# ejcanalesr/multicomponent-T2-toolbox

Hardware: AMD Instinct MI355X
Metric: voxels/sec (whole node) at nTE=32, nT2=60; max |MWF-ref| (higher is better)
Workload: dtype f64

## Files before the change

include/met2_hip.h:

```cpp
#ifndef MET2_HIP_H
#define MET2_HIP_H

#include <stdint.h>

#ifdef __cplusplus
extern "C" {
#endif

#define MET2_ABI_VERSION 6

enum met2_method {
    MET2_NNLS = 0,
    MET2_T2SPARC = 1,
    MET2_X2 = 2,
    MET2_LCURVE = 3,
    MET2_GCV = 4,
    MET2_BAYESREG = 5
};

enum met2_penalty { MET2_PEN_I = 0, MET2_PEN_L1 = 1, MET2_PEN_L2 = 2, MET2_PEN_INVT2 = 3 };

enum met2_status {
    MET2_ST_FITTED = 1,
    MET2_ST_ITMAX = 2,
// ... 229 lines not shown
int met2_tv_sigma(int32_t device, int32_t n_te, int64_t nc, const double *coef, const double *weight, double weight_factor, double *sigma,
                  double *weight_out, int32_t *copy, void *stream);

int met2_roi_reduce(met2_plan *src, met2_plan *dst, int64_t nvox, const double *data, int64_t voxel_stride, int64_t echo_stride,
                    const int32_t *roi_index, const double *fa_index, double *mean_signal, double *count, void *stream);

int met2_metrics(met2_plan *plan, int64_t nvox, const double *fsol, const uint8_t *mask, double *maps,
                 void *stream);

int met2_plan_last_kernel_ms(met2_plan *plan, double *ms);
int met2_plan_last_spill_count(met2_plan *plan, int64_t *count);
int met2_plan_last_second_pass_ms(met2_plan *plan, double *ms);

int met2_refac_packed_calls(met2_plan *plan, uint64_t *calls, int32_t reset);

int met2_plan_launch_info(met2_plan *plan, int32_t method, int32_t *grid, int32_t *block, int32_t *lds_bytes);

int met2_plan_gcv_form(met2_plan *plan, int32_t *low_rank, double *residual);

#ifdef __cplusplus
}
#endif
#endif
```

multicomponent-t2-toolbox_amd/_lib.py:

```python
import ctypes as C
import os

from . import _build

_LIB = None

_dp = C.POINTER(C.c_double)


class Met2Error(RuntimeError):
    pass


class Options(C.Structure):
    _fields_ = [("struct_size", C.c_int32), ("device", C.c_int32), ("x2_factor", C.c_double), ("t2sparc_lambda", C.c_double),
                ("brent_xtol", C.c_double), ("brent_maxfun", C.c_int32), ("reserved0", C.c_int32), ("t2_myelin_cut", C.c_double),
                ("t2_ie_cut", C.c_double), ("x2_lo", C.c_double), ("x2_hi", C.c_double), ("gcv_lo", C.c_double), ("gcv_hi", C.c_double),
                ("bayes_lo", C.c_double), ("bayes_hi", C.c_double)]


class SynthParams(C.Structure):
    _fields_ = [("struct_size", C.c_int32), ("reserved0", C.c_int32), ("te", C.c_double), ("TR", C.c_double), ("T1", C.c_double)] + [
        (k, C.c_double) for k in ("mwf_lo", "mwf_hi", "t2m_lo", "t2m_hi", "t2ie_lo", "t2ie_hi", "fa_lo", "fa_hi", "snr_lo", "snr_hi", "sm_lo", "sm_hi",
                                  "sie_lo", "sie_hi", "km")]


class TvGeometry(C.Structure):
    _fields_ = [(k, C.c_int32) for k in ("oy", "step1", "step2", "xlen", "nt1", "nt2", "nseg", "ntiles", "c0", "c1", "c2", "sigma_cap")] + [("nc", C.c_int64)]


SYMBOLS = ["met2_default_options", "met2_abi_version", "met2_device_count", "met2_last_error", "met2_plan_create",
           "met2_plan_destroy", "met2_plan_set_options", "met2_plan_get_options", "met2_plan_build_dictionary_epg", "met2_plan_set_dictionary", "met2_plan_get_dictionary",
           "met2_plan_set_penalty", "met2_plan_set_penalty_dense", "met2_plan_get_penalty", "met2_plan_set_lambda_grid",
           "met2_plan_set_t2_grid", "met2_fit", "met2_fit_strided", "met2_fit_enqueue_strided", "met2_plan_finish", "met2_fa_bruteforce", "met2_fa_bruteforce_strided", "met2_fa_spline_select",
           "met2_fa_spline_select_strided", "met2_roi_reduce", "met2_nesma", "met2_tv_work_bytes", "met2_tv_chambolle", "met2_tv_last_timing", "met2_tv_launch_info", "met2_tv_detail", "met2_tv_sigma", "met2_smooth_separable", "met2_metrics", "met2_plan_last_kernel_ms", "met2_plan_last_second_pass_ms", "met2_plan_last_spill_count",
           "met2_plan_launch_info", "met2_plan_gcv_form", "met2_plan_get_shape", "met2_fit_host", "met2_plan_attach_fa_spline", "met2_host_trim",
           "met2_fit_bootstrap", "met2_fit_bootstrap_fa", "met2_bootstrap_replicates", "met2_bootstrap_series_stats", "met2_bootstrap_spectrum_stats",
           "met2_bootstrap_spec_launch_info", "met2_synth_two_lobe", "met2_eval_voxel_metrics", "met2_eval_reduce", "met2_refac_packed_calls", "met2_mppca", "met2_mppca_stages", "met2_degibbs", "met2_bias_field",
           "met2_bias_weights", "met2_bias_domain", "met2_bias_init", "met2_bias_em", "met2_bias_smooth", "met2_bias_update", "met2_bias_apply",
           "met2_gibbs_table_cols", "met2_gibbs_tables", "met2_gibbs_split", "met2_gibbs_lines", "met2_degibbs3d", "met2_gibbs_split3d",
           "met2_brain_mask", "met2_bet_stats", "met2_bet_evolve", "met2_bet_fill", "met2_bet_mesh", "met2_bet_mean",
           "met2_tissue_segment", "met2_seg_consts", "met2_seg_init", "met2_seg_icm", "met2_seg_posterior", "met2_seg_finish",
           "met2_partial_volume", "met2_pve_moments", "met2_pve_consts", "met2_pve_energy", "met2_pve_icm", "met2_pve_finish"]


def lib():
    global _LIB
    if _LIB is None:
        path = _build.LIB
        if not os.path.exists(path):
            raise Met2Error("HIP extension %s is not built (run __graft_entry__.build()); there is no CPU fallback" % path)
        L = C.CDLL(path)
        L.met2_last_error.restype = C.c_char_p
# ... 59 lines not shown
        L.met2_pve_finish.argtypes = [C.c_int32, C.c_int64, vp, vp, C.c_int32, _dp, vp, vp, vp, vp]
        L.met2_tv_work_bytes.argtypes = [C.c_int32] * 5
        L.met2_tv_work_bytes.restype = C.c_int64
        L.met2_tv_chambolle.argtypes = [C.c_int32] * 5 + [vp, C.c_int32, _dp, C.c_double, C.c_double, C.c_int32, C.c_int32, vp, vp, vp, vp, C.c_int64, vp]
        L.met2_tv_last_timing.argtypes = [_dp, C.POINTER(C.c_int32)]
        L.met2_tv_launch_info.argtypes = [C.c_int32] * 5 + [C.POINTER(TvGeometry)]
        L.met2_tv_detail.argtypes = [C.c_int32] * 5 + [vp, C.c_int32, vp, vp]
        L.met2_tv_sigma.argtypes = [C.c_int32, C.c_int32, C.c_int64, vp, _dp, C.c_double, vp, vp, vp, vp]
        L.met2_smooth_separable.argtypes = [C.c_int32] * 6 + [_dp] + [vp] * 4
        L.met2_metrics.argtypes = [vp, C.c_int64, vp, vp, vp, vp]
        L.met2_plan_last_kernel_ms.argtypes = [vp, _dp]
        L.met2_plan_last_second_pass_ms.argtypes = [vp, _dp]
        L.met2_plan_last_spill_count.argtypes = [vp, C.POINTER(C.c_int64)]
        L.met2_plan_gcv_form.argtypes = [vp, C.POINTER(C.c_int32), _dp]
        L.met2_refac_packed_calls.argtypes = [vp, C.POINTER(C.c_uint64), C.c_int32]
        L.met2_plan_launch_info.argtypes = [vp, C.c_int32, C.POINTER(C.c_int32), C.POINTER(C.c_int32), C.POINTER(C.c_int32)]
        L.met2_plan_get_shape.argtypes = [vp, C.POINTER(C.c_int32), C.POINTER(C.c_int32), C.POINTER(C.c_int32)]
        L.met2_fit_host.argtypes = [C.POINTER(vp), C.c_int32, C.c_int32, C.c_int64, vp, vp, C.c_int64, C.c_int64, vp, vp, vp, C.c_int32] + [vp] * 8 + [C.c_int64, _dp]
        L.met2_host_trim.argtypes = []
        L.met2_plan_attach_fa_spline.argtypes = [vp, vp, C.c_int32, _dp, C.c_int32, _dp]
        L.met2_fit_bootstrap.argtypes = [vp, C.c_int32, C.c_int64, vp, C.c_int64, C.c_int64, vp, vp, vp, vp, C.c_int32, C.c_int64] + [vp] * 10
        L.met2_fit_bootstrap_fa.argtypes = [vp, C.c_int32, C.c_int32, C.c_int64, vp, C.c_int64, C.c_int64, vp, vp, vp, vp, C.c_int32, C.c_int64] + [vp] * 11
        L.met2_bootstrap_replicates.argtypes = [vp, C.c_int64, vp, vp, vp, C.c_int32, C.c_int64, vp, vp]
        L.met2_bootstrap_series_stats.argtypes = [C.c_int32, C.c_int64, C.c_int32, C.c_int32, vp, vp, vp, vp]
        L.met2_bootstrap_spectrum_stats.argtypes = [C.c_int32, C.c_int64, C.c_int32, C.c_int32, vp, vp, vp, vp]
        L.met2_bootstrap_spec_launch_info.argtypes = [C.c_int32, C.POINTER(C.c_int32), C.POINTER(C.c_int32), C.POINTER(C.c_int64)]
        L.met2_synth_two_lobe.argtypes = [vp, C.POINTER(SynthParams), C.c_int64, C.c_int64, C.c_int64, vp, vp, vp, vp]
        L.met2_eval_voxel_metrics.argtypes = [vp, C.c_int64, vp, vp, vp, vp]
        L.met2_eval_reduce.argtypes = [C.c_int64, vp, vp, vp, vp, vp, vp]
        _LIB = L
# ... 8 lines not shown
```

multicomponent-t2-toolbox_amd/csrc/fit_kernel.hpp:

```cpp
#pragma once
#include <hip/hip_runtime.h>
#include <math.h>
#include <stdint.h>

#include "../../include/met2_hip.h"
#include "abi_common.hpp"
#include "nnls_wave.hpp"
#include "objectives.hpp"

using namespace met2;

struct SortBufs {
    int *key;
    int *perm;
    int *hist;
    int *cursor;
    int *bucket_start;
    int *chunk_start;
    int *queue;
    int *xq;
    int *err;
    int *ovf;
};

// ... 30 lines not shown
    const char *seed;
    const double *btab;
    int nbtab, btab_stride;
    double *chol;
    int chol_stride;
    double *big;
    int big_stride;
    double *lc_save;
    int *lc_at;
    int lc_cap;
    double blam[MET2_BAYES_TABLE];
    int test_switches = 0;
    static constexpr int TEST_REFAC_PAIR = 1;
    static constexpr int TEST_SUBST_REF = 2;
    static constexpr int TEST_ROWWALK_REF = 4;
    unsigned long long *refac_count = nullptr;
};

#ifndef MET2_UNI_MASK
#define MET2_UNI_MASK 37
#endif
constexpr bool uni_brent(int method, int nb)
{
    const int base = method >= 10 ? method - 10 : method;
    const int bit = base == MET2_X2 ? 0 : ((base == MET2_GCV || base == MET2_GCV_LR) ? 2 : (base == MET2_BAYESREG ? 4 : -1));
    return bit >= 0 && ((MET2_UNI_MASK >> (bit + (nb == 2 ? 1 : 0))) & 1);
}
template <bool PIN>
__device__ __forceinline__ double uni(double v)
{
// ... 301 lines not shown
    if (base == MET2_BAYESREG) return (nb == 2) ? 8 : MET2_BAYES_WAVES;
    if (base <= MET2_LCURVE) return (nb == 2) ? 8 : 16;
    return 12;
}

struct SeedArgs {
    int n, m, nfa;
    const double *Dfa, *Bfa, *Dtfa, *kband, *lband, *Kd;
    double lam[4];
    char *out;
};
struct SeedRec {
    double x[128];
    int pos[128];
    int ord[128];
    int k, pad[3];
};

template <int NB>
__global__ __launch_bounds__(64) void seed_kernel(SeedArgs A)
{
    extern __shared__ __attribute__((aligned(16))) double smem[];
    const int lane = lane_id(), n = A.n, m = A.m, fa = (int)blockIdx.x, slot = (int)blockIdx.y;
    WaveShared S;
    S.R = smem; S.n = n; S.m = m; S.kmax = n; S.rcap = col_base(n); S.K = A.Kd; S.kband = A.kband;
    S.B = A.Bfa + (size_t)fa * n * n; S.D = A.Dfa + (size_t)fa * m * n; S.Dt = A.Dtfa + (size_t)fa * m * n; S.DtG = S.Dt;
    S.bstride = n; S.dstride = n; S.dtstride = m; S.buffer_rows = true; S.reorder = true; S.have_bdiag = false; S.bdiag[0] = S.bdiag[1] = 0.0;
    Band<NB> bd;
    load_band<NB>(bd, A.kband, A.lband, lane);
    double b = 0.0;
    for (int j = 0; j < n; ++j) {
        const double u = (double)j / (double)(n - 1), d1 = (u - 0.13) / 0.05, d2 = (u - 0.39) / 0.05;
        const double xc = 0.15 * exp(-0.5 * d1 * d1) + 0.85 * exp(-0.5 * d2 * d2);
        if (lane < m) b = fma(S.Dt[(size_t)j * m + lane], xc, b);
    }
    b = b / bcast(b, 0);
    NnlsState<NB> st; st.itmax_hit = 0;
    MET2_CYC_INIT(st);
    nnls_reset<NB>(st);
    project<NB>(S, b, lane, st.h);
    nnls_solve<NB>(S, bd, st, A.lam[slot], true, lane);
    SeedRec *rec = (SeedRec *)A.out + ((size_t)slot * A.nfa + fa);
#pragma unroll
    for (int bb = 0; bb < NB; ++bb) {
        rec->x[lane + 64 * bb] = st.x[bb];
        rec->pos[lane + 64 * bb] = st.pos[bb];
        rec->ord[lane + 64 * bb] = st.ord[bb];
    }
    if (lane == 0) rec->k = (st.itmax_hit == 0) ? st.k : 0;
}

struct BayesTabArgs {
    int n, m, nfa, nj, stride;
    const double *Bfa, *Kd, *kband, *lband;
    double lam[MET2_BAYES_TABLE > 0 ? MET2_BAYES_TABLE : 1];
    double *out;
};
template <int NB>
__global__ __launch_bounds__(64) void bayes_table_kernel(BayesTabArgs A)
{
    extern __shared__ __attribute__((aligned(16))) double smem[];
    const int lane = lane_id(), n = A.n, fa = (int)blockIdx.x, j = (int)blockIdx.y;
    WaveShared S;
    S.R = smem; S.n = n; S.m = A.m; S.kmax = n; S.rcap = col_base(n); S.K = A.Kd; S.kband = A.kband;
// ... 22 lines not shown
{
    const __amdgpu_buffer_rsrc_t r = __builtin_amdgcn_make_buffer_rsrc((void *)seed, 0, 0x40000000, 0x00020000);
    const unsigned rec = (unsigned)fa * (unsigned)sizeof(SeedRec);
#pragma unroll
    for (int b = 0; b < NB; ++b) {
        const unsigned e = (unsigned)(lane + 64 * b);
        const auto xv = __builtin_amdgcn_raw_buffer_load_b64(r, 8u * e, rec, 0);
        st.x[b] = __hiloint2double((int)xv[1], (int)xv[0]);
        st.pos[b] = (int)__builtin_amdgcn_raw_buffer_load_b32(r, 4u * e, rec + (unsigned)offsetof(SeedRec, pos), 0);
        st.ord[b] = (int)__builtin_amdgcn_raw_buffer_load_b32(r, 4u * e, rec + (unsigned)offsetof(SeedRec, ord), 0);
        st.P[b] = ballot(st.pos[b] >= 0);
    }
    st.k = k;
}

template <int NB, int ONE, bool BIG>
__device__ __forceinline__ void solve_warm(const WaveShared &S, const Band<NB> &bd, NnlsState<NB> &st, double lam, bool aug, int lane)
{
    if constexpr (BIG) { NnlsState<NB> sc = st; big_solve_fn<NB, ONE>(S, (big_lds_dp)S.R, bd, &sc, lam, (aug ? 1 : 0) | 2); st = sc; }
    else nnls_solve_warm<NB, ONE>(S, bd, st, lam, aug, lane);
}
template <int NB, int ONE, bool BIG>
__device__ __forceinline__ void solve_cold(const WaveShared &S, const Band<NB> &bd, NnlsState<NB> &st, double lam, bool aug, int lane)
{
    if constexpr (BIG) { NnlsState<NB> sc = st; big_solve_fn<NB, ONE>(S, (big_lds_dp)S.R, bd, &sc, lam, aug ? 1 : 0); st = sc; }
    else nnls_solve<NB, ONE>(S, bd, st, lam, aug, lane);
}
template <int NB, bool BIG>
__device__ __forceinline__ void refine(const WaveShared &S, NnlsState<NB> &st, double lam, double bvec, int lane)
{
    if constexpr (BIG) { NnlsState<NB> sc = st; big_refine_fn<NB>(S, (big_lds_dp)S.R, &sc, lam, bvec); st = sc; }
    else refine_csne<NB>(S, st, lam, bvec, lane);
}

template <int METHOD, int NB, bool BIG>
__device__ __forceinline__ bool fit_voxel(const FitArgs &A, const WaveShared &S, const Band<NB> &bd, const MetricLanes<NB> &ml, int64_t v, int fa,
                                          int seed_k, bool have_seed, int lane, int wslot, int qslot)
{
    constexpr int ONE = (NB == 2) ? (((METHOD >= 10 ? METHOD - 10 : METHOD) <= MET2_LCURVE) ? 1 : MET2_ONE_REFAC) : 0;
    const int n = A.n, m = A.m;
    double b = (lane < m) ? A.data[v * A.vs + lane * A.es] : 0.0;
    const double km = bcast(b, 0);
    b = b / km;
    NnlsState<NB> st; st.itmax_hit = 0;
    MET2_CYC_INIT(st);
    MET2_CYC_BEGIN(c_vox);
    nnls_reset<NB>(st);
    project<NB>(S, b, lane, st.h);
    double regv = 0.0, lamv = 0.0; int stat = MET2_ST_FITTED;
    bool queued = false;

    if (METHOD == MET2_NNLS) {
        solve_cold<NB, ONE, BIG>(S, bd, st, 0.0, false, lane);
    } else if (METHOD == MET2_T2SPARC) {
        if (have_seed) { seed_load<NB>(st, A.seed, seed_k, fa, lane); solve_warm<NB, ONE, BIG>(S, bd, st, A.t2sparc_lambda, true, lane); }
        else solve_cold<NB, ONE, BIG>(S, bd, st, A.t2sparc_lambda, true, lane);
        regv = lamv = A.t2sparc_lambda;
    } else if (METHOD == MET2_X2) {
        solve_cold<NB, ONE, BIG>(S, bd, st, 0.0, false, lane);
        constexpr bool PIN = uni_brent(METHOD, NB);
        const double SSE = uni<PIN>(sse_of<NB>(S, st, b, lane));
        const double target = uni<PIN>(A.x2_factor * SSE);
        int flag;
        double last_x = -1.0, last_sse = 0.0;
        if (have_seed) seed_load<NB>(st, A.seed, seed_k, fa, lane);
        double best_x[NB], best_sse = 0.0; int best_pos[NB], best_ord[NB];
#ifdef MET2_CYCSTATS
        int evi = 0; double canon = 0.0;
#endif
#if MET2_TIE_GUARD
// ... 370 lines not shown
```

multicomponent-t2-toolbox_amd/csrc/met2_fit_nnls_lcurve.hip:

```cpp
#ifdef MET2_SPLIT_TU
#define MET2_REFAC_PACKED 1
#define MET2_ROWWALK 1
#include "fit_kernel.hpp"
template int launch_fit_nb<0, 1, false>(const FitArgs &, const LaunchGeom &, hipStream_t);
template int launch_fit_nb<0, 2, false>(const FitArgs &, const LaunchGeom &, hipStream_t);
template int launch_fit_nb<1, 1, false>(const FitArgs &, const LaunchGeom &, hipStream_t);
template int launch_fit_nb<1, 2, false>(const FitArgs &, const LaunchGeom &, hipStream_t);
template int launch_fit_nb<3, 1, false>(const FitArgs &, const LaunchGeom &, hipStream_t);
template int launch_fit_nb<3, 2, false>(const FitArgs &, const LaunchGeom &, hipStream_t);
template int launch_fit_nb<0, 1, true>(const FitArgs &, const LaunchGeom &, hipStream_t);
template int launch_fit_nb<0, 2, true>(const FitArgs &, const LaunchGeom &, hipStream_t);
template int launch_fit_nb<1, 1, true>(const FitArgs &, const LaunchGeom &, hipStream_t);
template int launch_fit_nb<1, 2, true>(const FitArgs &, const LaunchGeom &, hipStream_t);
template int launch_fit_nb<3, 1, true>(const FitArgs &, const LaunchGeom &, hipStream_t);
template int launch_fit_nb<3, 2, true>(const FitArgs &, const LaunchGeom &, hipStream_t);
#endif
```

multicomponent-t2-toolbox_amd/csrc/met2_hip.hip:

```cpp
#include <hip/hip_runtime.h>
#include <math.h>
#include <stddef.h>
#include <stdint.h>
#include <stdio.h>
#include <stdlib.h>
#include <string.h>
#include <string>
#include <vector>

#include "../../include/met2_hip.h"
#include "abi_common.hpp"
#include "nnls_wave.hpp"
#include "objectives.hpp"
#include "fit_kernel.hpp"

using namespace met2;

#ifdef MET2_SPLIT_TU
extern template int launch_fit_nb<0, 1, false>(const FitArgs &, const LaunchGeom &, hipStream_t);
extern template int launch_fit_nb<0, 2, false>(const FitArgs &, const LaunchGeom &, hipStream_t);
extern template int launch_fit_nb<1, 1, false>(const FitArgs &, const LaunchGeom &, hipStream_t);
extern template int launch_fit_nb<1, 2, false>(const FitArgs &, const LaunchGeom &, hipStream_t);
extern template int launch_fit_nb<2, 1, false>(const FitArgs &, const LaunchGeom &, hipStream_t);
extern template int launch_fit_nb<2, 2, false>(const FitArgs &, const LaunchGeom &, hipStream_t);
// ... 805 lines not shown
    __syncthreads();
    const double nv = s_nv;
    if ((int)threadIdx.x < A.nte) {
        double t = 0.0;
        for (int sl = 0; sl < A.nslice; ++sl) t += A.part_sig[((size_t)r * A.nslice + sl) * 64 + threadIdx.x];
        A.mean_sig[(size_t)r * A.nte + threadIdx.x] = t / nv;
    }
    const int sz = A.nte * A.nt2;
    for (int i = threadIdx.x; i < sz; i += blockDim.x) {
        double t = 0.0;
        for (int f = 0; f < A.nfa; ++f) { const int c = roi_tot[f]; if (c) t = fma((double)c, A.Dsrc[(size_t)f * sz + i], t); }
        A.Ddst[(size_t)r * sz + i] = t / nv;
    }
}

__device__ unsigned long long g_refac_packed_calls;

struct met2_plan {
    int n_te, n_t2, n_fa;
    met2_options opt;
    int cus;
    double *dD = nullptr;
    double *dB = nullptr;
    double *dKband = nullptr;
    double *dLband = nullptr;
    double *dDt = nullptr;
    double *dKd = nullptr;
    double *dLam = nullptr;
    double *dT2 = nullptr;
    int nlam = 0;
    bool have_dict = false, have_pen = false, have_t2 = false;
// ... 480 lines not shown
    hipDeviceProp_t prop;
    HIPCHK(hipGetDeviceProperties(&prop, p->opt.device));
    p->cus = prop.multiProcessorCount;
    HIPCHK(hipMalloc(&p->dD, sizeof(double) * (size_t)n_fa * n_te * n_t2));
    HIPCHK(hipMalloc(&p->dB, sizeof(double) * (size_t)n_fa * n_t2 * n_t2));
    HIPCHK(hipMalloc(&p->dDt, sizeof(double) * (size_t)n_fa * n_te * n_t2));
    HIPCHK(hipMalloc(&p->dAq, sizeof(double) * (size_t)n_fa * n_t2 * MET2_GCV_LR_RANK));
    HIPCHK(hipMalloc(&p->dAqRes, sizeof(double) * (size_t)n_fa));
    HIPCHK(hipMalloc(&p->dQt, sizeof(double) * (size_t)n_fa * MET2_GCV_LR_RANK * n_te));
    HIPCHK(hipMalloc(&p->dKband, sizeof(double) * 5 * 128));
    HIPCHK(hipMalloc(&p->dLband, sizeof(double) * 5 * 128));
    HIPCHK(hipMalloc(&p->dKd, sizeof(double) * (size_t)n_t2 * n_t2));
    HIPCHK(hipMemset(p->dKd, 0, sizeof(double) * (size_t)n_t2 * n_t2));
    HIPCHK(hipMalloc(&p->dT2, sizeof(double) * 128));
    HIPCHK(hipMalloc(&p->dSmall, sizeof(int) * (4 * (size_t)(n_fa + 1) + 16)));
    HIPCHK(hipMalloc(&p->dSeed, sizeof(SeedRec) * 4 * (size_t)n_fa));
    HIPCHK(hipHostMalloc((void **)&p->hErr, 4 * sizeof(int), hipHostMallocDefault));
    p->hErr[0] = p->hErr[1] = p->hErr[2] = p->hErr[3] = 0;
    HIPCHK(hipEventCreate(&p->ev0));
    HIPCHK(hipEventCreate(&p->ev1));
    HIPCHK(hipEventCreate(&p->ev2));
    std::vector<double> g;
    default_lambda_grid(g);
    *out = p;
    return met2_plan_set_lambda_grid(p, g.data(), (int)g.size());
}

int met2_plan_set_options(met2_plan *p, const met2_options *opt)
{
    if (!p || !opt) return fail(MET2_E_INVALID, "NULL argument");
    if (opt->device != p->opt.device) return fail(MET2_E_INVALID, "a plan cannot change device");
// ... 354 lines not shown
    }

    FitArgs A;
    A.n = p->n_t2; A.m = p->n_te; A.nfa = p->n_fa; A.kmax = g.kmax; A.waves = g.waves; A.chunk = chunk; A.wave_doubles = g.wave_doubles;
    A.method = method; A.nlam = p->nlam;
    A.maxfun = p->opt.brent_maxfun > 0 ? p->opt.brent_maxfun : (method == MET2_BAYESREG ? 200 : 300);
    A.x2_factor = p->opt.x2_factor; A.t2sparc_lambda = p->opt.t2sparc_lambda; A.xtol = p->opt.brent_xtol;
    A.cut_m = p->opt.t2_myelin_cut; A.cut_ie = p->opt.t2_ie_cut;
    A.lam_lo = method == MET2_GCV ? p->opt.gcv_lo : (method == MET2_BAYESREG ? p->opt.bayes_lo : p->opt.x2_lo);
    A.lam_hi = method == MET2_GCV ? p->opt.gcv_hi : (method == MET2_BAYESREG ? p->opt.bayes_hi : p->opt.x2_hi);
    A.log_detL = p->log_detL;
    A.Dfa = p->dD; A.Bfa = p->dB; A.Dtfa = p->dDt; A.Aq = p->dAq; A.kband = p->dKband; A.lband = p->dLband; A.Kd = p->dKd; A.lam_grid = p->dLam; A.t2s = p->dT2;
    A.data = data; A.vs = voxel_stride; A.es = echo_stride; A.sb = sb; A.fsol = fsol; A.sig = sig; A.reg = reg; A.lam = lam; A.maps = maps; A.status = status; A.nvox = nvox;

    A.test_switches = (test_switch("MET2_REFAC_PAIR") ? FitArgs::TEST_REFAC_PAIR : 0) | (test_switch("MET2_SUBST_REF") ? FitArgs::TEST_SUBST_REF : 0) |
                      (test_switch("MET2_ROWWALK_REF") ? FitArgs::TEST_ROWWALK_REF : 0);
    A.refac_count = nullptr;
    if (test_switch("MET2_REFAC_COUNT")) HIPCHK(hipGetSymbolAddress((void **)&A.refac_count, HIP_SYMBOL(g_refac_packed_calls)));
    A.seed = nullptr;
    if (!test_switch("MET2_NO_SEED") && !objgrid && p->have_pen && p->seeds_valid && p->seeds_ok && p->seeds_key[0] == p->opt.t2sparc_lambda &&
        (method == MET2_X2 || method == MET2_GCV || method == MET2_BAYESREG || method == MET2_T2SPARC)) {
        const int slot = method == MET2_BAYESREG ? 1 : (method == MET2_T2SPARC ? 2 : (method == MET2_GCV ? 3 : 0));
        A.seed = p->dSeed + sizeof(SeedRec) * (size_t)slot * p->n_fa;
    }
    A.btab = nullptr; A.nbtab = 0; A.btab_stride = p->btab_stride;
    A.chol = nullptr; A.chol_stride = 0;
    if (method == MET2_BAYESREG && !objgrid && g.nb == 2) {
        const int stride = (col_base(p->n_t2) + 15) & ~15;
        const int64_t need = (int64_t)g.grid * g.waves * stride;
        if (p->cap_chol < need) {
            if (p->dChol) { HIPCHK(hipStreamSynchronize(s)); HIPCHK(hipFree(p->dChol)); p->dChol = nullptr; p->cap_chol = 0; }
            HIPCHK(hipMalloc(&p->dChol, sizeof(double) * (size_t)need));
            p->cap_chol = need;
        }
        A.chol = p->dChol; A.chol_stride = stride;
    }
    A.big = nullptr; A.big_stride = 0;
    if (kfast) {
// ... 250 lines not shown
    return MET2_OK;
}

int met2_refac_packed_calls(met2_plan *p, uint64_t *calls, int32_t reset)
{
    if (!p) return fail(MET2_E_INVALID, "NULL plan");
    USE_DEVICE(p->opt.device);
    HIPCHK(hipDeviceSynchronize());
    unsigned long long v = 0;
    HIPCHK(hipMemcpyFromSymbol(&v, HIP_SYMBOL(g_refac_packed_calls), sizeof(v)));
    if (calls) *calls = (uint64_t)v;
    if (reset) { v = 0; HIPCHK(hipMemcpyToSymbol(HIP_SYMBOL(g_refac_packed_calls), &v, sizeof(v))); }
    return MET2_OK;
}

int met2_plan_launch_info(met2_plan *p, int32_t method, int32_t *grid, int32_t *block, int32_t *lds_bytes)
{
    if (!p) return fail(MET2_E_INVALID, "NULL plan");
    LaunchGeom g;
    method = kernel_method(p, method);
    const int kf = fast_kmax(p, method);
    int rc = fit_geometry(p, method, g, kf);
    if (rc) return rc;
    if (grid) *grid = g.grid;
    if (block) *block = g.block;
    if (lds_bytes) *lds_bytes = g.lds;
    return MET2_OK;
}

}
// ... 1 lines not shown
```

multicomponent-t2-toolbox_amd/csrc/nnls_wave.hpp:

```cpp
#pragma once
#include "wave_ops.hpp"

namespace met2 {

#ifndef MET2_DOUBLE
#define MET2_DOUBLE 0
#endif
#ifndef MET2_REORDER
#define MET2_REORDER 2
#endif

#ifdef MET2_LOOPSTATS
__device__ int g_loopstats[8];
#define MET2_STAT(slot, v) atomicMax(&g_loopstats[slot], (int)(v))
#else
#define MET2_STAT(slot, v)
#endif

#ifdef MET2_CYCSTATS
__device__ unsigned long long g_cyc[16];
__device__ unsigned long long g_ev[40][12];
__device__ unsigned long long g_refk[4];
#define MET2_CYC_BEGIN(var) const unsigned long long var = __builtin_readcyclecounter()
#define MET2_CYC_END(slot, var) st.cyc[slot] += __builtin_readcyclecounter() - var
// ... 343 lines not shown
#pragma unroll
    for (int b = 0; b < NP; ++b) ordn[b] = (NP == 1) ? gather_i(st.ord[0], (lane + 1) & 63) : gatherN_i<NB>(st.ord, lane + 64 * b + 1);
#pragma unroll
    for (int b = 0; b < NB; ++b) {
        const int pl = lane + 64 * b;
        if (b < NP) st.ord[b] = (pl >= p) ? ordn[b] : st.ord[b];
        st.pos[b] = (st.pos[b] > p) ? st.pos[b] - 1 : st.pos[b];
        if (pl == tb) { st.pos[b] = -1; st.x[b] = 0.0; }
    }
    clear_bit<NB>(st.P, tb);
    st.k = k - 1;
    MET2_CYC_END(7, c_rm);
    MET2_CYC_ADD(6, 1);
}

template <int NB, int NP = NB>
__device__ __forceinline__ bool try_append(const WaveShared &S, const Band<NB> &bd, NnlsState<NB> &st, double lam, int t, int lane,
                                           bool forced = false)
{
    const int k = st.k;
    double gb[NB];
#pragma unroll
    for (int b = 0; b < NB; ++b) {
        const int j = lane + 64 * b;
        const unsigned je = (unsigned)min(j, S.n - 1);
        const double bv = ld_row_sel(S.buffer_rows, S.B, t * S.bstride, je);
        gb[b] = (j < S.n) ? bv : 0.0;
        if (lam != 0.0) gb[b] = fma(lam, (j < S.n) ? ld_row_sel(S.buffer_rows, S.K, t * S.n, je) : 0.0, gb[b]);
    }
    const double gtt = bcastN<NB>(gb, t);
    double g[NB], rv[NB];
    int cbl[NB];
#pragma unroll
    for (int b = 0; b < NP; ++b) {
        const int pl = lane + 64 * b;
        cbl[b] = col_base(pl);
        double gg = gatherN<NB>(gb, st.ord[b]);
        g[b] = (pl < k) ? gg : 0.0;
        rv[b] = (k > 0 && pl > 0 && pl < k) ? S.R[cbl[b]] : 0.0;
    }
    bool lean = false;
    if constexpr (NB == 1 && NP == 1) lean = !S.subst_ref;
    if (lean) {
        const u64 kmask = k >= 64 ? ~0ull : (1ull << k) - 1ull;
        const double *col = S.R + cbl[0];
        double gq = g[0], ru = rv[0], rw = 0.0;
        const double rinv = st.rinv[0];
        for (int i = 0; i + 1 < k; i += 2) {
            double s = bcast(gq * rinv, i);
            if (lane_in(kmask & (~1ull << i))) { gq = fma(-ru, s, gq); rw = col[i + 1]; }
            s = bcast(gq * rinv, i + 1);
            if (lane_in(kmask & (~3ull << i))) { gq = fma(-rw, s, gq); ru = col[i + 2]; }
        }
        g[0] = gq;
    } else {
        double rw[NB];
#pragma unroll
        for (int b = 0; b < NP; ++b) rw[b] = 0.0;
        int i = 0;
        for (; i + 1 < k; i += 2) {
#pragma unroll
            for (int b = 0; b < NP; ++b) { const int pl = lane + 64 * b; rw[b] = (pl > i + 1 && pl < k) ? S.R[cbl[b] + i + 1] : 0.0; }
            {
                double tt = (NP == 2 && (i >> 6)) ? g[NB - 1] * st.rinv[NB - 1] : g[0] * st.rinv[0];
                double s = bcast(tt, i & 63);
#pragma unroll
                for (int b = 0; b < NP; ++b) g[b] = fma(-rv[b], s, g[b]);
            }
#pragma unroll
// ... 307 lines not shown
            if (S.Rg) iterate_big<NB>(S, bd, st, lam, mrows, lane, warm, iter, outer);
        } else
            (void)iterate_leg<NB, NB>(S, bd, st, lam, mrows, lane, warm, iter, outer);
    } else
        nnls_iterate_plain<NB, (NB == 2 && ONE == 3), BIG>(S, bd, st, lam, mrows, lane, warm);
}

template <int NB>
__device__ __forceinline__ void nnls_reset(NnlsState<NB> &st)
{
#pragma unroll
    for (int b = 0; b < NB; ++b) { st.x[b] = 0.0; st.y[b] = 0.0; st.rinv[b] = 0.0; st.ord[b] = 0; st.pos[b] = -1; st.P[b] = 0ull; }
    st.k = 0;
}

template <int NB, int NP = NB, bool PACK = false>
__device__ __forceinline__ bool refactor_rowwise(const WaveShared &S, const Band<NB> &bd, NnlsState<NB> &st, double lam, int lane)
{
    static_assert(!PACK || (NB == 1 && NP == 1), "the packed leg is written for one bin per lane");
    const int k = st.k, n = S.n;
#ifdef MET2_CYCSTATS
    if (lane == 0) {
        const unsigned long long terms = (unsigned long long)(k * (k - 1) / 2);
        atomicAdd(&g_refk[0], 1ull); atomicAdd(&g_refk[1], terms);
        if (k > 32) { atomicAdd(&g_refk[2], 1ull); atomicAdd(&g_refk[3], terms); }
    }
#endif
    int cbl[NB], cbc[NB];
    unsigned jc[NB];
    double g[NB], gb0[NB], gk0[NB], gb1[NB], gk1[NB];
#pragma unroll
    for (int b = 0; b < NB; ++b) {
        const int pl = lane + 64 * b;
        jc[b] = (unsigned)min(pl, n - 1);
// ... 8 lines not shown
        const int t = bcastPos_i<NB, NP>(st.ord, min(p, k - 1));
#pragma unroll
        for (int b = 0; b < NB; ++b) {
            vb[b] = ld_row_sel(S.buffer_rows, S.B, t * S.bstride, jc[b]);
            vk[b] = ld_row_sel(S.buffer_rows, S.K, t * n, jc[b]);
        }
    };
    auto finish = [&](int i, double (&a)[NB], double (&r)[NB]) {
        const double d = bcastPos<NB, NP>(a, i);
        const double rinv = rsqrt_nr(d);
        const double yi = bcastPos<NB, NP>(g, i) * rinv;
#pragma unroll
        for (int b = 0; b < NP; ++b) {
            const int pl = lane + 64 * b;
            r[b] = a[b] * rinv;
            if (pl >= i && pl < k) S.R[cbl[b] + i] = r[b];
            g[b] = (pl > i) ? fma(-r[b], yi, g[b]) : g[b];
        }
    };
    double gdp[NB];
    {
        double gdb[NB];
#pragma unroll
        for (int b = 0; b < NB; ++b) {
            const double bd0 = S.have_bdiag ? S.bdiag[b] : S.B[jc[b] * S.bstride + jc[b]];
            gdb[b] = (lam != 0.0) ? fma(lam, S.K[jc[b] * n + jc[b]], bd0) : bd0;
        }
#pragma unroll
        for (int b = 0; b < NP; ++b) gdp[b] = gatherN<NB>(gdb, st.ord[b]);
    }
// ... 469 lines not shown
            const int t = bcastN_i<NB>(ordold, p);
            bool okp;
            if constexpr (BIG) okp = (st.k >= S.kmax) ? try_append_big<NB>(S, bd, st, lam, t, lane, true) : try_append<NB>(S, bd, st, lam, t, lane, true);
            else okp = try_append<NB>(S, bd, st, lam, t, lane, true);
            if (!okp) {
#pragma unroll
                for (int b = 0; b < NB; ++b) if (lane + 64 * b == t) st.x[b] = 0.0;
            }
        }
    }
    MET2_CYC_END(1, c_ref);
    MET2_CYC_ADD(12, 1);
    nnls_iterate<NB, ONE, BIG>(S, bd, st, lam, aug ? S.m + S.n : S.m, lane, true);
}

template <int NB>
__device__ __forceinline__ double model_signal(const WaveShared &S, const NnlsState<NB> &st, int lane)
{
    const int k = st.k;
    double acc = 0.0, acc2 = 0.0, xp[NB];
#pragma unroll
    for (int b = 0; b < NB; ++b) { const double t = gatherN<NB>(st.x, st.ord[b]); xp[b] = (lane + 64 * b < k) ? t : 0.0; }
    if constexpr (NB == 1 && MET2_ROWWALK_ON(2)) if (S.m <= 32 && S.buffer_rows && !S.rowwalk_ref) {
        const int lo_ = lane_opaque(lane), hi = lo_ >> 5;
        const unsigned ecb = 8u * (unsigned)min(lo_ & 31, S.m - 1), rowb = 8u * (unsigned)S.dtstride;
#pragma clang loop unroll(disable)
        for (int p = 0; p < k; p += 4) {
            const int pa = p + hi, pb = pa + 2;
            const unsigned ta = (unsigned)gather_i(st.ord[0], pa), tb = (unsigned)gather_i(st.ord[0], pb);
            const double va = ld_row(S.Dt, 0, ta * rowb + ecb), vb = ld_row(S.Dt, 0, tb * rowb + ecb);
// ... 230 lines not shown
```

Baseline: 7.713 million.

## Store seed Cholesky factors and reuse them in T2SPARC warm-start solves

The seed kernel now also computes the Cholesky factor of the seed active set, with row scales and inverse diagonals, and stores it next to each per-flip-angle seed record. In T2SPARC fits with one bin per lane, the warm start loads this stored factor into LDS and runs only a forward substitution, skipping a full row-wise refactorization for every voxel. The cost is larger seed buffers, extra global loads per voxel, and more work in the seed kernel. Other methods and multi-bin paths keep the old warm start.

Result: no change. 7.714 million (median of 3 runs) (+0.0%).

```diff
diff --git a/include/met2_hip.h b/include/met2_hip.h
--- a/include/met2_hip.h
+++ b/include/met2_hip.h
@@ -267,6 +267,10 @@
 
 int met2_refac_packed_calls(met2_plan *plan, uint64_t *calls, int32_t reset);
 
+int met2_seed_factor_calls(met2_plan *plan, uint64_t *calls, int32_t reset);
+
+int met2_plan_seed_info(met2_plan *plan, int32_t method, int32_t fa, int32_t *k, int32_t *has_factor);
+
 int met2_plan_launch_info(met2_plan *plan, int32_t method, int32_t *grid, int32_t *block, int32_t *lds_bytes);
 
 int met2_plan_gcv_form(met2_plan *plan, int32_t *low_rank, double *residual);
diff --git a/multicomponent-t2-toolbox_amd/_lib.py b/multicomponent-t2-toolbox_amd/_lib.py
--- a/multicomponent-t2-toolbox_amd/_lib.py
+++ b/multicomponent-t2-toolbox_amd/_lib.py
@@ -36,7 +36,7 @@
            "met2_fa_spline_select_strided", "met2_roi_reduce", "met2_nesma", "met2_tv_work_bytes", "met2_tv_chambolle", "met2_tv_last_timing", "met2_tv_launch_info", "met2_tv_detail", "met2_tv_sigma", "met2_smooth_separable", "met2_metrics", "met2_plan_last_kernel_ms", "met2_plan_last_second_pass_ms", "met2_plan_last_spill_count",
            "met2_plan_launch_info", "met2_plan_gcv_form", "met2_plan_get_shape", "met2_fit_host", "met2_plan_attach_fa_spline", "met2_host_trim",
            "met2_fit_bootstrap", "met2_fit_bootstrap_fa", "met2_bootstrap_replicates", "met2_bootstrap_series_stats", "met2_bootstrap_spectrum_stats",
-           "met2_bootstrap_spec_launch_info", "met2_synth_two_lobe", "met2_eval_voxel_metrics", "met2_eval_reduce", "met2_refac_packed_calls", "met2_mppca", "met2_mppca_stages", "met2_degibbs", "met2_bias_field",
+           "met2_bootstrap_spec_launch_info", "met2_synth_two_lobe", "met2_eval_voxel_metrics", "met2_eval_reduce", "met2_refac_packed_calls", "met2_seed_factor_calls", "met2_plan_seed_info", "met2_mppca", "met2_mppca_stages", "met2_degibbs", "met2_bias_field",
            "met2_bias_weights", "met2_bias_domain", "met2_bias_init", "met2_bias_em", "met2_bias_smooth", "met2_bias_update", "met2_bias_apply",
            "met2_gibbs_table_cols", "met2_gibbs_tables", "met2_gibbs_split", "met2_gibbs_lines", "met2_degibbs3d", "met2_gibbs_split3d",
            "met2_brain_mask", "met2_bet_stats", "met2_bet_evolve", "met2_bet_fill", "met2_bet_mesh", "met2_bet_mean",
@@ -126,6 +126,8 @@
         L.met2_plan_last_spill_count.argtypes = [vp, C.POINTER(C.c_int64)]
         L.met2_plan_gcv_form.argtypes = [vp, C.POINTER(C.c_int32), _dp]
         L.met2_refac_packed_calls.argtypes = [vp, C.POINTER(C.c_uint64), C.c_int32]
+        L.met2_seed_factor_calls.argtypes = [vp, C.POINTER(C.c_uint64), C.c_int32]
+        L.met2_plan_seed_info.argtypes = [vp, C.c_int32, C.c_int32, C.POINTER(C.c_int32), C.POINTER(C.c_int32)]
         L.met2_plan_launch_info.argtypes = [vp, C.c_int32, C.POINTER(C.c_int32), C.POINTER(C.c_int32), C.POINTER(C.c_int32)]
         L.met2_plan_get_shape.argtypes = [vp, C.POINTER(C.c_int32), C.POINTER(C.c_int32), C.POINTER(C.c_int32)]
         L.met2_fit_host.argtypes = [C.POINTER(vp), C.c_int32, C.c_int32, C.c_int64, vp, vp, C.c_int64, C.c_int64, vp, vp, vp, C.c_int32] + [vp] * 8 + [C.c_int64, _dp]
diff --git a/multicomponent-t2-toolbox_amd/csrc/fit_kernel.hpp b/multicomponent-t2-toolbox_amd/csrc/fit_kernel.hpp
--- a/multicomponent-t2-toolbox_amd/csrc/fit_kernel.hpp
+++ b/multicomponent-t2-toolbox_amd/csrc/fit_kernel.hpp
@@ -68,6 +68,7 @@
     static constexpr int TEST_REFAC_PAIR = 1;
     static constexpr int TEST_SUBST_REF = 2;
     static constexpr int TEST_ROWWALK_REF = 4;
+    static constexpr int TEST_SEED_FACTOR_REF = 8;
     unsigned long long *refac_count = nullptr;
 };
 
@@ -399,8 +400,13 @@
     double x[128];
     int pos[128];
     int ord[128];
-    int k, pad[3];
+    int k;
+    int fac;
+    int pad[2];
 };
+__host__ __device__ constexpr int seed_factor_doubles(int n) { return n <= 64 ? col_base(n) + 2 * n : 0; }
+__host__ __device__ constexpr size_t seed_slot_bytes(int n, int nfa) { return (size_t)nfa * (sizeof(SeedRec) + sizeof(double) * (size_t)seed_factor_doubles(n)); }
+constexpr int SEED_PAD_DOUBLES = 256;
 
 template <int NB>
 __global__ __launch_bounds__(64) void seed_kernel(SeedArgs A)
@@ -425,7 +431,8 @@
     nnls_reset<NB>(st);
     project<NB>(S, b, lane, st.h);
     nnls_solve<NB>(S, bd, st, A.lam[slot], true, lane);
-    SeedRec *rec = (SeedRec *)A.out + ((size_t)slot * A.nfa + fa);
+    char *slot_base = A.out + (size_t)slot * seed_slot_bytes(n, A.nfa);
+    SeedRec *rec = (SeedRec *)slot_base + fa;
 #pragma unroll
     for (int bb = 0; bb < NB; ++bb) {
         rec->x[lane + 64 * bb] = st.x[bb];
@@ -433,6 +440,21 @@
         rec->ord[lane + 64 * bb] = st.ord[bb];
     }
     if (lane == 0) rec->k = (st.itmax_hit == 0) ? st.k : 0;
+    bool fac = false;
+    if constexpr (NB == 1) {
+        if (st.itmax_hit == 0 && st.k > 0) {
+            const int k = st.k;
+            double scales[1] = {0.0};
+            __builtin_amdgcn_wave_barrier();
+            fac = refactor_rowwise<1, 1, false, true>(S, bd, st, A.lam[slot], lane, &scales);
+            __builtin_amdgcn_wave_barrier();
+            double *frec = (double *)(slot_base + (size_t)A.nfa * sizeof(SeedRec)) + (size_t)fa * seed_factor_doubles(n);
+            const int tri = col_base(k);
+            for (int i = lane; i < tri; i += 64) frec[i] = smem[i];
+            if (lane < k) { frec[col_base(n) + lane] = scales[0]; frec[col_base(n) + n + lane] = st.rinv[0]; }
+        }
+    }
+    if (lane == 0) rec->fac = fac ? 1 : 0;
 }
 
 struct BayesTabArgs {
@@ -485,6 +507,42 @@
     st.k = k;
 }
 
+#if !defined(MET2_SEED_FACTOR) && !defined(MET2_SPLIT_TU)
+#define MET2_SEED_FACTOR 1
+#endif
+#ifndef MET2_SEED_FACTOR
+#define MET2_SEED_FACTOR 0
+#endif
+__device__ __forceinline__ void seed_factor_load(const WaveShared &S, NnlsState<1> &st, const char *seed, int nfa, int fa, int lane)
+{
+    const int k = st.k, n = S.n, tri = col_base(k);
+    const __amdgpu_buffer_rsrc_t r = __builtin_amdgcn_make_buffer_rsrc((void *)seed, 0, 0x40000000, 0x00020000);
+    const unsigned rec = (unsigned)nfa * (unsigned)sizeof(SeedRec) + (unsigned)fa * (unsigned)(sizeof(double) * seed_factor_doubles(n));
+    const unsigned rs = rec + 8u * (unsigned)col_base(n);
+    const auto sv = __builtin_amdgcn_raw_buffer_load_b64(r, 8u * (unsigned)lane, rs, 0);
+    const auto iv = __builtin_amdgcn_raw_buffer_load_b64(r, 8u * (unsigned)lane, rs + 8u * (unsigned)n, 0);
+    for (int i0 = 0; i0 < tri; i0 += 256) {
+        const unsigned e = (unsigned)(i0 + lane);
+        const auto v0 = __builtin_amdgcn_raw_buffer_load_b64(r, 8u * e, rec, 0);
+        const auto v1 = __builtin_amdgcn_raw_buffer_load_b64(r, 8u * e, rec + 512u, 0);
+        const auto v2 = __builtin_amdgcn_raw_buffer_load_b64(r, 8u * e, rec + 1024u, 0);
+        const auto v3 = __builtin_amdgcn_raw_buffer_load_b64(r, 8u * e, rec + 1536u, 0);
+        double *d = S.R + e;
+        if ((int)e < tri) d[0] = __hiloint2double((int)v0[1], (int)v0[0]);
+        if ((int)e + 64 < tri) d[64] = __hiloint2double((int)v1[1], (int)v1[0]);
+        if ((int)e + 128 < tri) d[128] = __hiloint2double((int)v2[1], (int)v2[0]);
+        if ((int)e + 192 < tri) d[192] = __hiloint2double((int)v3[1], (int)v3[0]);
+    }
+    __builtin_amdgcn_wave_barrier();
+    const double scale = __hiloint2double((int)sv[1], (int)sv[0]), rinv = __hiloint2double((int)iv[1], (int)iv[0]);
+    const double hh = gatherN<1>(st.h, st.ord[0]);
+    const double *col = S.R + col_base(lane);
+    const double ru = (lane > 0 && lane < k) ? col[0] : 0.0;
+    const double g = forward_lean(col, (lane < k) ? hh : 0.0, ru, scale, k);
+    st.rinv[0] = (lane < k) ? rinv : st.rinv[0];
+    st.y[0] = (lane < k) ? g * rinv : st.y[0];
+}
+
 template <int NB, int ONE, bool BIG>
 __device__ __forceinline__ void solve_warm(const WaveShared &S, const Band<NB> &bd, NnlsState<NB> &st, double lam, bool aug, int lane)
 {
@@ -496,6 +554,18 @@
 {
     if constexpr (BIG) { NnlsState<NB> sc = st; big_solve_fn<NB, ONE>(S, (big_lds_dp)S.R, bd, &sc, lam, aug ? 1 : 0); st = sc; }
     else nnls_solve<NB, ONE>(S, bd, st, lam, aug, lane);
+}
+constexpr bool seed_factor_leg(int method, int nb, bool big) { return MET2_SEED_FACTOR && nb == 1 && !big && method == MET2_T2SPARC; }
+template <int NB, int ONE>
+__device__ __forceinline__ void solve_first(const FitArgs &A, const WaveShared &S, const Band<NB> &bd, NnlsState<NB> &st, double lam, int fa, int lane)
+{
+    static_assert(NB == 1, "the factor records exist at one bin per lane");
+    nnls_solve_warm_with<NB, ONE>(S, bd, st, lam, true, lane, [&]() {
+        if (((const SeedRec *)A.seed)[fa].fac == 0 || (A.test_switches & FitArgs::TEST_SEED_FACTOR_REF) != 0) return false;
+        seed_factor_load(S, st, A.seed, A.nfa, fa, lane);
+        if (A.refac_count && lane == 0) atomicAdd(A.refac_count + 1, 1ull);
+        return true;
+    });
 }
 template <int NB, bool BIG>
 __device__ __forceinline__ void refine(const WaveShared &S, NnlsState<NB> &st, double lam, double bvec, int lane)
@@ -524,7 +594,11 @@
     if (METHOD == MET2_NNLS) {
         solve_cold<NB, ONE, BIG>(S, bd, st, 0.0, false, lane);
     } else if (METHOD == MET2_T2SPARC) {
-        if (have_seed) { seed_load<NB>(st, A.seed, seed_k, fa, lane); solve_warm<NB, ONE, BIG>(S, bd, st, A.t2sparc_lambda, true, lane); }
+        if (have_seed) {
+            seed_load<NB>(st, A.seed, seed_k, fa, lane);
+            if constexpr (seed_factor_leg(METHOD, NB, BIG)) solve_first<NB, ONE>(A, S, bd, st, A.t2sparc_lambda, fa, lane);
+            else solve_warm<NB, ONE, BIG>(S, bd, st, A.t2sparc_lambda, true, lane);
+        }
         else solve_cold<NB, ONE, BIG>(S, bd, st, A.t2sparc_lambda, true, lane);
         regv = lamv = A.t2sparc_lambda;
     } else if (METHOD == MET2_X2) {
diff --git a/multicomponent-t2-toolbox_amd/csrc/met2_fit_nnls_lcurve.hip b/multicomponent-t2-toolbox_amd/csrc/met2_fit_nnls_lcurve.hip
--- a/multicomponent-t2-toolbox_amd/csrc/met2_fit_nnls_lcurve.hip
+++ b/multicomponent-t2-toolbox_amd/csrc/met2_fit_nnls_lcurve.hip
@@ -1,6 +1,7 @@
 #ifdef MET2_SPLIT_TU
 #define MET2_REFAC_PACKED 1
 #define MET2_ROWWALK 1
+#define MET2_SEED_FACTOR 1
 #include "fit_kernel.hpp"
 template int launch_fit_nb<0, 1, false>(const FitArgs &, const LaunchGeom &, hipStream_t);
 template int launch_fit_nb<0, 2, false>(const FitArgs &, const LaunchGeom &, hipStream_t);
diff --git a/multicomponent-t2-toolbox_amd/csrc/met2_hip.hip b/multicomponent-t2-toolbox_amd/csrc/met2_hip.hip
--- a/multicomponent-t2-toolbox_amd/csrc/met2_hip.hip
+++ b/multicomponent-t2-toolbox_amd/csrc/met2_hip.hip
@@ -843,7 +843,7 @@
     }
 }
 
-__device__ unsigned long long g_refac_packed_calls;
+__device__ unsigned long long g_refac_packed_calls[2];
 
 struct met2_plan {
     int n_te, n_t2, n_fa;
@@ -1354,7 +1354,7 @@
     HIPCHK(hipMemset(p->dKd, 0, sizeof(double) * (size_t)n_t2 * n_t2));
     HIPCHK(hipMalloc(&p->dT2, sizeof(double) * 128));
     HIPCHK(hipMalloc(&p->dSmall, sizeof(int) * (4 * (size_t)(n_fa + 1) + 16)));
-    HIPCHK(hipMalloc(&p->dSeed, sizeof(SeedRec) * 4 * (size_t)n_fa));
+    HIPCHK(hipMalloc(&p->dSeed, 4 * seed_slot_bytes(n_t2, n_fa) + sizeof(double) * SEED_PAD_DOUBLES));
     HIPCHK(hipHostMalloc((void **)&p->hErr, 4 * sizeof(int), hipHostMallocDefault));
     p->hErr[0] = p->hErr[1] = p->hErr[2] = p->hErr[3] = 0;
     HIPCHK(hipEventCreate(&p->ev0));
@@ -1739,14 +1739,14 @@
     A.data = data; A.vs = voxel_stride; A.es = echo_stride; A.sb = sb; A.fsol = fsol; A.sig = sig; A.reg = reg; A.lam = lam; A.maps = maps; A.status = status; A.nvox = nvox;
 
     A.test_switches = (test_switch("MET2_REFAC_PAIR") ? FitArgs::TEST_REFAC_PAIR : 0) | (test_switch("MET2_SUBST_REF") ? FitArgs::TEST_SUBST_REF : 0) |
-                      (test_switch("MET2_ROWWALK_REF") ? FitArgs::TEST_ROWWALK_REF : 0);
+                      (test_switch("MET2_ROWWALK_REF") ? FitArgs::TEST_ROWWALK_REF : 0) | (test_switch("MET2_SEED_FACTOR_REF") ? FitArgs::TEST_SEED_FACTOR_REF : 0);
     A.refac_count = nullptr;
     if (test_switch("MET2_REFAC_COUNT")) HIPCHK(hipGetSymbolAddress((void **)&A.refac_count, HIP_SYMBOL(g_refac_packed_calls)));
     A.seed = nullptr;
     if (!test_switch("MET2_NO_SEED") && !objgrid && p->have_pen && p->seeds_valid && p->seeds_ok && p->seeds_key[0] == p->opt.t2sparc_lambda &&
         (method == MET2_X2 || method == MET2_GCV || method == MET2_BAYESREG || method == MET2_T2SPARC)) {
         const int slot = method == MET2_BAYESREG ? 1 : (method == MET2_T2SPARC ? 2 : (method == MET2_GCV ? 3 : 0));
-        A.seed = p->dSeed + sizeof(SeedRec) * (size_t)slot * p->n_fa;
+        A.seed = p->dSeed + seed_slot_bytes(p->n_t2, p->n_fa) * (size_t)slot;
     }
     A.btab = nullptr; A.nbtab = 0; A.btab_stride = p->btab_stride;
     A.chol = nullptr; A.chol_stride = 0;
@@ -2027,6 +2027,35 @@
     return MET2_OK;
 }
 
+int met2_seed_factor_calls(met2_plan *p, uint64_t *calls, int32_t reset)
+{
+    if (!p) return fail(MET2_E_INVALID, "NULL plan");
+    USE_DEVICE(p->opt.device);
+    HIPCHK(hipDeviceSynchronize());
+    unsigned long long v = 0;
+    HIPCHK(hipMemcpyFromSymbol(&v, HIP_SYMBOL(g_refac_packed_calls), sizeof(v), sizeof(v)));
+    if (calls) *calls = (uint64_t)v;
+    if (reset) { v = 0; HIPCHK(hipMemcpyToSymbol(HIP_SYMBOL(g_refac_packed_calls), &v, sizeof(v), sizeof(v))); }
+    return MET2_OK;
+}
+
+int met2_plan_seed_info(met2_plan *p, int32_t method, int32_t fa, int32_t *k, int32_t *has_factor)
+{
+    if (!p) return fail(MET2_E_INVALID, "NULL plan");
+    if (fa < 0 || fa >= p->n_fa) return fail(MET2_E_INVALID, "flip-angle index outside the plan");
+    if (method != MET2_X2 && method != MET2_GCV && method != MET2_BAYESREG && method != MET2_T2SPARC) return fail(MET2_E_INVALID, "the method has no seed");
+    USE_DEVICE(p->opt.device);
+    int kf[2] = {0, 0};
+    if (p->seeds_valid && p->seeds_ok) {
+        const int slot = method == MET2_BAYESREG ? 1 : (method == MET2_T2SPARC ? 2 : (method == MET2_GCV ? 3 : 0));
+        HIPCHK(hipDeviceSynchronize());
+        HIPCHK(hipMemcpy(kf, p->dSeed + seed_slot_bytes(p->n_t2, p->n_fa) * (size_t)slot + sizeof(SeedRec) * (size_t)fa + offsetof(SeedRec, k), sizeof(kf), hipMemcpyDeviceToHost));
+    }
+    if (k) *k = kf[0];
+    if (has_factor) *has_factor = kf[0] > 0 ? kf[1] : 0;
+    return MET2_OK;
+}
+
 int met2_plan_launch_info(met2_plan *p, int32_t method, int32_t *grid, int32_t *block, int32_t *lds_bytes)
 {
     if (!p) return fail(MET2_E_INVALID, "NULL plan");
diff --git a/multicomponent-t2-toolbox_amd/csrc/nnls_wave.hpp b/multicomponent-t2-toolbox_amd/csrc/nnls_wave.hpp
--- a/multicomponent-t2-toolbox_amd/csrc/nnls_wave.hpp
+++ b/multicomponent-t2-toolbox_amd/csrc/nnls_wave.hpp
@@ -381,6 +381,19 @@
     MET2_CYC_ADD(6, 1);
 }
 
+__device__ __forceinline__ double forward_lean(const double *col, double gq, double ru, double scale, int k)
+{
+    const u64 kmask = k >= 64 ? ~0ull : (1ull << k) - 1ull;
+    double rw = 0.0;
+    for (int i = 0; i + 1 < k; i += 2) {
+        double s = bcast(gq * scale, i);
+        if (lane_in(kmask & (~1ull << i))) { gq = fma(-ru, s, gq); rw = col[i + 1]; }
+        s = bcast(gq * scale, i + 1);
+        if (lane_in(kmask & (~3ull << i))) { gq = fma(-rw, s, gq); ru = col[i + 2]; }
+    }
+    return gq;
+}
+
 template <int NB, int NP = NB>
 __device__ __forceinline__ bool try_append(const WaveShared &S, const Band<NB> &bd, NnlsState<NB> &st, double lam, int t, int lane,
                                            bool forced = false)
@@ -409,17 +422,7 @@
     bool lean = false;
     if constexpr (NB == 1 && NP == 1) lean = !S.subst_ref;
     if (lean) {
-        const u64 kmask = k >= 64 ? ~0ull : (1ull << k) - 1ull;
-        const double *col = S.R + cbl[0];
-        double gq = g[0], ru = rv[0], rw = 0.0;
-        const double rinv = st.rinv[0];
-        for (int i = 0; i + 1 < k; i += 2) {
-            double s = bcast(gq * rinv, i);
-            if (lane_in(kmask & (~1ull << i))) { gq = fma(-ru, s, gq); rw = col[i + 1]; }
-            s = bcast(gq * rinv, i + 1);
-            if (lane_in(kmask & (~3ull << i))) { gq = fma(-rw, s, gq); ru = col[i + 2]; }
-        }
-        g[0] = gq;
+        g[0] = forward_lean(S.R + cbl[0], g[0], rv[0], st.rinv[0], k);
     } else {
         double rw[NB];
 #pragma unroll
@@ -757,10 +760,12 @@
     st.k = 0;
 }
 
-template <int NB, int NP = NB, bool PACK = false>
-__device__ __forceinline__ bool refactor_rowwise(const WaveShared &S, const Band<NB> &bd, NnlsState<NB> &st, double lam, int lane)
+template <int NB, int NP = NB, bool PACK = false, bool SCALES = false>
+__device__ __forceinline__ bool refactor_rowwise(const WaveShared &S, const Band<NB> &bd, NnlsState<NB> &st, double lam, int lane,
+                                                 double (*scales)[NB] = nullptr)
 {
     static_assert(!PACK || (NB == 1 && NP == 1), "the packed leg is written for one bin per lane");
+    static_assert(!SCALES || !PACK, "the row scales are handed out by the pair loop");
     const int k = st.k, n = S.n;
 #ifdef MET2_CYCSTATS
     if (lane == 0) {
@@ -799,6 +804,7 @@
         for (int b = 0; b < NP; ++b) {
             const int pl = lane + 64 * b;
             r[b] = a[b] * rinv;
+            if constexpr (SCALES) { if (pl == i) (*scales)[b] = rinv; }
             if (pl >= i && pl < k) S.R[cbl[b] + i] = r[b];
             g[b] = (pl > i) ? fma(-r[b], yi, g[b]) : g[b];
         }
@@ -1298,6 +1304,15 @@
     nnls_iterate<NB, ONE, BIG>(S, bd, st, lam, aug ? S.m + S.n : S.m, lane, true);
 }
 
+template <int NB, int ONE = 0, class F>
+__device__ __forceinline__ void nnls_solve_warm_with(const WaveShared &S, const Band<NB> &bd, NnlsState<NB> &st, double lam, bool aug, int lane, F &&plan_factor)
+{
+    if (st.k > 0 && plan_factor()) {
+        MET2_CYC_ADD(12, 1);
+        nnls_iterate<NB, ONE, false>(S, bd, st, lam, aug ? S.m + S.n : S.m, lane, true);
+    } else nnls_solve_warm<NB, ONE, false>(S, bd, st, lam, aug, lane);
+}
+
 template <int NB>
 __device__ __forceinline__ double model_signal(const WaveShared &S, const NnlsState<NB> &st, int lane)
 {
```
